# PengfeiRen96/DIR

Measured on AMD Instinct MI355X. Metric: images/sec at 256x256 bs=64, 3 stage outputs (DIR.forward eval), higher is better.
Workload: dtype f16

## Files before the change

dir_amd/_capi.py:

```python
import ctypes as C
import os

_HERE = os.path.dirname(os.path.abspath(__file__))
LIB_PATH = os.environ.get('DIR_LIB_PATH') or os.path.join(_HERE, 'lib', 'libdir_hip.so')
_lib = None


class DirHipError(RuntimeError):
    pass


class ManoTables(C.Structure):
    _fields_ = [('shapedirs_t', C.c_void_p), ('posedirs_t', C.c_void_p), ('v_template', C.c_void_p),
                ('j_template', C.c_void_p), ('j_shapedirs', C.c_void_p), ('weights', C.c_void_p), ('hands_mean', C.c_void_p),
                ('comps', C.c_void_p), ('side', C.c_int32), ('center_idx', C.c_int32), ('root_palm', C.c_int32)]


class ConvDesc(C.Structure):
    _fields_ = [(n, C.c_int32) for n in (
        'B', 'H', 'W', 'Cin', 'in_cstride', 'in_coff', 'Cout', 'out_cstride', 'out_coff', 'res_cstride', 'res_coff',
        'kh', 'kw', 'stride', 'pad', 'in_dtype', 'out_dtype', 'flags', 'Ho', 'Wo')] + [('in_scale', C.c_float), ('out_split_scale', C.c_float)]


class ConvBnBwd(C.Structure):
    _fields_ = [(n, C.c_void_p) for n in ('z', 'mean', 'rstd', 'w', 'b')] + [('relu', C.c_int32)] + [(n, C.c_void_p) for n in ('p1', 'p2')]


class ConvSrc2(C.Structure):
    _fields_ = [(n, C.c_int32) for n in ('H', 'W', 'Cin', 'in_cstride', 'in_coff', 'stride')]


class TrainWeight(C.Structure):
    _fields_ = [(n, C.c_void_p) for n in ('w', 'fwd', 'fwd_scale', 'dgrad', 'dgrad_scale')] + [(n, C.c_int32) for n in ('Cout', 'Cin', 'kh', 'kw')] + [
        ('fwd_inv_in', C.c_float), ('dgrad_inv_in', C.c_float)]


class BneckChainParams(C.Structure):
    _fields_ = [(n, C.c_void_p) for n in ('w2', 'scale2', 'shift2', 'w3', 'scale3', 'shift3', 'w1n', 'scale1n', 'shift1n', 'wd')] + [
        ('n_next', C.c_int32), ('out_decimate', C.c_int32), ('dtype', C.c_int32)]


class BneckTailParams(C.Structure):
    _fields_ = [(n, C.c_void_p) for n in ('wstream', 'scale3', 'shift3', 'scale1n', 'shift1n')] + [('planes', C.c_int32), ('n_next', C.c_int32), ('waves', C.c_int32), ('dtype', C.c_int32)]


class GemmDesc(C.Structure):
    _fields_ = [(n, C.c_int32) for n in ('M', 'N', 'K', 'lda', 'ldb', 'ldc', 'trans_a', 'trans_b', 'accumulate', 'batch')] + \
               [(n, C.c_int64) for n in ('stride_a', 'stride_b', 'stride_c')]


class GemmGroups(C.Structure):
    _fields_ = [(n, C.c_int32) for n in ('ny', 'nx', 'reduce', 'reserved')] + [(n, C.c_int64) for n in ('a_y', 'a_x', 'b_y', 'b_x', 'c_y', 'c_x')]


class TokenMlp(C.Structure):
    _fields_ = [(n, C.c_void_p) for n in ('w1t', 's1', 'b1', 'w2t', 'b2')]


class PgcnLayer(C.Structure):
    _fields_ = [(n, C.c_void_p) for n in ('W', 'e1', 'bias', 'bn_scale', 'bn_shift')] + [('relu', C.c_int32), ('w_dtype', C.c_int32)]


class SteBlock(C.Structure):
    _fields_ = [(n, C.c_void_p) for n in ('ln1_w', 'ln1_b', 'qkv_wt', 'qkv_b', 'proj_wt', 'proj_b', 'ln2_w', 'ln2_b',
                                          'fc1_wt', 'fc1_b', 'fc2_wt', 'fc2_b')]


class SteParams(C.Structure):
# ... 22 lines not shown


class LossPred(C.Structure):
    _fields_ = [('joint_uv', C.c_void_p * 2), ('mesh_uv', C.c_void_p * 2), ('proj', C.c_void_p * 2), ('joint_xyz', C.c_void_p * 2),
                ('mesh_xyz', C.c_void_p * 2), ('offset', C.c_void_p)]


class LossTarget(C.Structure):
    _fields_ = [('joint_2d', C.c_void_p * 2), ('mesh_2d', C.c_void_p * 2), ('joint_3d', C.c_void_p * 2),
                ('mesh_3d', C.c_void_p * 2), ('center', C.c_void_p * 2), ('faces', C.c_void_p * 2),
                ('c2', C.c_int32), ('n_faces', C.c_int32)]


class LossPredGrad(C.Structure):
    _fields_ = [('joint_uv', C.c_void_p * 2), ('mesh_uv', C.c_void_p * 2), ('joint_xyz', C.c_void_p * 2),
                ('mesh_xyz', C.c_void_p * 2), ('offset', C.c_void_p)]


class EvalOutputs(C.Structure):
    _fields_ = [(n, C.c_void_p) for n in ('joint_err', 'vert_err', 'joint2d_err', 'vert2d_err', 'joints_pd', 'joints_gt',
                                          'root_err')]


ABI_VERSION = 39
DT_F32, DT_BF16, DT_F16X3, DT_F16X1, DT_F16X3P, DT_F16X1P, DT_F16 = 0, 1, 3, 4, 5, 6, 7
CONV_RELU, CONV_PRE_RELU = 1, 2

_p, _i = C.c_void_p, C.c_int
_SIGNATURES = {
    'dir_abi_version': (C.c_int, []),
    'dir_last_error': (C.c_char_p, []),
    'dir_device_info': (C.c_int, [C.c_char_p, _i, C.POINTER(C.c_int)]),
    'dir_launch_log_reset': (None, []),
    'dir_launch_log_get': (C.c_int, [C.c_char_p, _i]),
    'dir_launch_log_note': (None, [C.c_char_p, C.c_longlong]),
    'dir_probe_launch': (C.c_longlong, [_i, _p, C.c_longlong, _i, _p]),
    'dir_conv2d_forward': (C.c_int, [C.POINTER(ConvDesc), _p, _p, _p, _p, _p, _p, _p, _p, _p]),
    'dir_conv2d_forward_stats': (C.c_int, [C.POINTER(ConvDesc), _p, _p, _p, _p, _p, _p, _p, _p, _p, C.POINTER(C.c_int), _p]),
    'dir_conv2d_forward_masked': (C.c_int, [C.POINTER(ConvDesc), _p, _p, _p, _p, _p, _p, _p, _p, _p, _p]),
    'dir_conv2d_forward_ex': (C.c_int, [C.POINTER(ConvDesc), _p, _p, _p, _p, _p, _p, _p, _p, _p, C.POINTER(ConvBnBwd), C.POINTER(C.c_int), _p]),
    'dir_add_upsampled': (C.c_int, [_p, _p, _i, _i, _i, _i, _i, _i, _i, _p]),
    'dir_fuse_sum': (C.c_int, [_p, _p, _p, _p, _i, _i, _i, _i, _i, _i, _i, _p]),
    'dir_pack_f16x3_weights': (C.c_int, [_p, _p, _p, _p, _i, _i, _p]),
    'dir_train_pack_conv_weights': (C.c_int, [_p, _p, _i, _i, _p]),
    'dir_gemm_f32_splitk_workspace_bytes': (C.c_longlong, [C.POINTER(GemmDesc)]),
    'dir_gemm_f32_splitk': (C.c_int, [C.POINTER(GemmDesc), _p, _p, _p, _p, _p, C.c_longlong, _p]),
    'dir_axpy_multi_f32': (C.c_int, [_p, _p, _p, _i, C.c_float, _p]),
    'dir_split_f16_forward': (C.c_int, [_p, _p, C.c_longlong, _i, _i, _i, _p, _p, _i, C.c_float, _i, _p]),
    'dir_stem_prep': (C.c_int, [_p, _p, _i, _i, _i, _i, _i, _i, _i, _p]),
    'dir_stem_prep_s2d': (C.c_int, [_p, _p, _i, _i, _i, _i, _i, _i, _p]),
    'dir_image_normalize_forward': (C.c_int, [_p, _p, C.POINTER(C.c_float), C.POINTER(C.c_float), _i, _i, _i, _p]),
    'dir_stem_prep_s2d_u8': (C.c_int, [_p, _p, C.POINTER(C.c_float), C.POINTER(C.c_float), _i, _i, _i, _i, _i, _i, _p]),
    'dir_adamw_step': (C.c_int, [_p, _p, _p, _p, C.c_longlong, C.c_double, C.c_double, C.c_double, C.c_double, C.c_double,
                                 C.c_longlong, _p]),
    'dir_stage_losses_backward': (C.c_int, [C.POINTER(LossPred), C.POINTER(LossTarget), C.c_float, _p, C.POINTER(C.c_void_p * 2),
                                            C.POINTER(C.c_void_p * 2), C.POINTER(LossPredGrad), _i, _p]),
    'dir_dense_losses_backward_workspace_bytes': (C.c_longlong, [_i, _i]),
    'dir_dense_losses_backward': (C.c_int, [_p, _p, _p, _p, C.POINTER(C.c_float), C.c_float, _p, _p, C.c_longlong, _p, _p, _i, _i, _i, _i, _p]),
    'dir_stage_losses_forward': (C.c_int, [C.POINTER(LossPred), C.POINTER(LossTarget), C.c_float, _p, _p, _i, _p]),
    'dir_dense_losses_workspace_bytes': (C.c_longlong, [_i, _i]),
    'dir_dense_losses_forward': (C.c_int, [_p, _p, _p, _p, C.POINTER(C.c_float), C.c_float, _p, C.c_longlong, _p, _i, _i, _i, _i, _p]),
    'dir_bottleneck_chain_forward': (C.c_int, [C.POINTER(BneckChainParams), _p, _p, _p, _p, _p, _i, _i, _i, _p]),
    'dir_bottleneck_tail_forward': (C.c_int, [C.POINTER(BneckTailParams), _p, _p, _p, _p, C.c_longlong, _p]),
    'dir_stem_pool_forward': (C.c_int, [_p, _i, C.POINTER(C.c_float), C.POINTER(C.c_float), _p, _p, _p, _p, _i, _i, _i, _p]),
    'dir_stem_pool_forward_dt': (C.c_int, [_p, _i, _i, C.POINTER(C.c_float), C.POINTER(C.c_float), _p, _p, _p, _p, _i, _i, _i, _p]),
    'dir_maxpool3x3s2': (C.c_int, [_p, _p, _i, _i, _i, _i, _i, _p]),
    'dir_upsample2x_bilinear': (C.c_int, [_p, _p, _i, _i, _i, _i, _i, _i, _i, _p]),
    'dir_init_head_forward': (C.c_int, [C.POINTER(InitHeadParams), _p, _p, _p, _i, _p, _p, _p, _i, _i, _i, _i, _i, _p]),
    'dir_bone_proj_forward': (C.c_int, [_p, _p, _p, _p, _p, _p, _i, _i, C.c_float, _i, _p]),
    'dir_conv2d_dual_forward': (C.c_int, [C.POINTER(ConvDesc), _p, C.POINTER(ConvSrc2), _p, _p, _p, _p, _p]),
    'dir_conv2d_dual_scaled_forward': (C.c_int, [C.POINTER(ConvDesc), _p, C.POINTER(ConvSrc2), _p, _p, _p, _p, _p, _p]),
    'dir_conv1x1_stream_forward': (C.c_int, [C.POINTER(ConvDesc), _p, C.POINTER(ConvSrc2), _p, _p, _p, _p, _p, _p, _p, _p]),
    'dir_conv2d_as_supported': (C.c_int, [C.POINTER(ConvDesc), _i, _i]),
    'dir_conv2d_as_forward': (C.c_int, [C.POINTER(ConvDesc), _p, _p, _p, _p, _p, _p, _i, _i, _p]),
    'dir_conv2d_sparse_forward': (C.c_int, [C.POINTER(ConvDesc), _p, _p, _p, _p, _p, _p, _p, _p]),
    'dir_grid_tokens_forward': (C.c_int, [_p, _i, _i, _i, _i, _i, _p, _p, _p, _p, _p, C.POINTER(TokenMlp),
                                          C.POINTER(TokenMlp), C.POINTER(TokenMlp), _p, _p, _i, _p]),
    'dir_pgcn_stack_forward': (C.c_int, [C.POINTER(PgcnLayer), _i, _p, _p, _p, C.c_longlong, _p, _i, _p]),
    'dir_pgcn_stack_forward_pair': (C.c_int, [C.POINTER(PgcnLayer), C.POINTER(PgcnLayer), _i, _p, _p, _p, _p, _i, _p]),
    'dir_pgcn_fused_sync_bytes': (C.c_longlong, []),
    'dir_pgcn_stack_forward_fused': (C.c_int, [C.POINTER(PgcnLayer), C.POINTER(PgcnLayer), _i, _p, _p, _p, _p, _p, _i, _i, _p]),
    'dir_ste_forward': (C.c_int, [C.POINTER(SteParams), _p, _p, _p, _i, _p]),
    'dir_regress_forward': (C.c_int, [C.POINTER(RegressParams), _p, _p, _p, _p, _p, _p, _p, _p, _i, _p]),
    'dir_bone_fusion_scratch_bytes': (C.c_size_t, [_i]),
    'dir_bone_fusion_prepare': (C.c_int, [C.POINTER(BoneFusionParams), _p, _p, _i, _p]),
    'dir_bone_fusion_forward': (C.c_int, [C.POINTER(BoneFusionParams), _p, _p, _p, _p, _i, _i, C.c_float, _i, _i, _i, _p]),
# ... 154 lines not shown
```

dir_amd/engine.py:

```python
import ctypes as C
import math
import json
import os
import threading

import torch

from . import _capi
from ._capi import CONV_PRE_RELU, CONV_RELU, DT_BF16, DT_F16, DT_F16X1, DT_F16X1P, DT_F16X3, DT_F16X3P, DT_F32, ConvDesc

F32 = torch.float32
IMAGENET_MEAN = (C.c_float * 3)(0.485, 0.456, 0.406)
IMAGENET_STD = (C.c_float * 3)(0.229, 0.224, 0.225)
_TLS = threading.local()


def _forced_variant():
    return getattr(_TLS, 'variant', None)


def _packing_arith():
    return getattr(_TLS, 'arith', None)


# ... 472 lines not shown
                and c1n.kh == 1 and c1n.stride == 1 and c1n.cin == c3.cout and c1n.scale is not None and c1n.pre_scale is None
                and (c3.cin, c1n.cout) in BneckTailOp.GEOMETRIES)

    def __call__(self, y2, x, out=None, y1n=None):
        B, H, W, P = y2.shape
        M = B * H * W
        if getattr(_TLS, 'capture_fused', None) is not None:
            _TLS.capture_fused.append((self, (y2, x), {}))
        if out is None:
            out = torch.empty(B, H, W, self.c3.cout, device=y2.device, dtype=y2.dtype)
        if y1n is None:
            y1n = torch.empty(B, H, W, self.c1n.cout, device=y2.device, dtype=y2.dtype)
        if _capi.PROFILE is not None:
            c4, n2 = self.c3.cout, self.c1n.cout
            _capi.annotate(family='conv', flops=2.0 * M * (P * c4 + c4 * n2), op=self, dtype='bf16',
                           shape='M=%d tail 1x1(%d->%d)+res+1x1(->%d)' % (M, P, c4, n2),
                           bytes=(M * (P + 2 * c4 + n2) + c4 * P + n2 * c4) * 2)
        waves = self.force_waves or (4 if M // 64 <= self.THIN_MAX_TILES else 8)
        _capi.check(_capi.lib().dir_bottleneck_tail_forward(C.byref(self.params[waves]), _capi.ptr(y2), _capi.ptr(x), _capi.ptr(out), _capi.ptr(y1n),
                                                            M, _capi.stream_ptr()), 'dir_bottleneck_tail_forward')
        return out, y1n


def stem_conv_op(w, scale, shift, dtype):
    wp = torch.zeros(64, 64, 4, 1, device=w.device, dtype=F32)
    for r in range(4):
        for dy in range(2):
            ky = 2 * r + dy - 1
            if not 0 <= ky <= 6:
                continue
            for j in range(4):
                for dx in range(2):
                    kx = 2 * j + dx - 1
                    if 0 <= kx <= 6:
                        c0 = j * 16 + (dy * 2 + dx) * 4
                        wp[:, c0:c0 + 3, r, 0] = w[:, :, ky, kx]
    op = ConvOp(wp, dtype, stride=1, pad=0, scale=scale, shift=shift, relu=True)
    op.ho = op.wo = 128
    op.in_cs_override = 16
    op.alg_k = 147
    return op


class BackboneOp(object):
    fold_downsample = os.environ.get('DIR_FOLD_DOWNSAMPLE', '1') != '0'
    fused_stem = os.environ.get('DIR_FUSED_STEM', '1') != '0'
# ... 32 lines not shown
                if 'dual' not in blk and blk['ds'] is None:
                    blk['c2'].link_split(blk['c3'])
                blocks.append(blk)
            self.layers.append(blocks)
        if self.bneck_chain:
            l1 = self.layers[0]
            for i, blk in enumerate(l1):
                nxt = l1[i + 1]['c1'] if i + 1 < len(l1) else self.layers[1][0]['c1']
                if 'dual' in blk:
                    if BneckChainOp.applies(blk['c2'], None, nxt, dt, dual=blk['dual']):
                        blk['chain'] = BneckChainOp(blk['c2'], None, nxt, dual=blk['dual'])
                elif blk['ds'] is None and BneckChainOp.applies(blk['c2'], blk['c3'], nxt, dt):
                    blk['chain'] = BneckChainOp(blk['c2'], blk['c3'], nxt)

        if self.bneck_tail:
            for li in (1, 2):
                blocks = self.layers[li]
                for i, blk in enumerate(blocks):
                    if 'dual' in blk or blk['ds'] is not None or 'chain' in blk:
                        continue
                    nxt = blocks[i + 1]['c1'] if i + 1 < len(blocks) else self.layers[li + 1][0]['c1']
                    if BneckTailOp.applies(blk['c3'], nxt, dt):
                        blk['tail'] = BneckTailOp(blk['c3'], nxt)

    def __call__(self, img):
        L, dt, dev = _capi.lib(), self.dtype, self.device
        B = img.shape[0]
        if self.fused_stem and dt in HALF:
            x = torch.empty(B, 64, 64, 64, device=dev, dtype=dt)
            u8 = img.dtype == torch.uint8
            _ann('stem', 2.0 * B * 128 * 128 * 64 * 147, img.numel() * img.element_size() + x.numel() * 2 + self.stem_w.numel() * 2,
                 'B=%d 7x7/2 conv + bn + relu + maxpool' % B)
            nb = self.subbatch
            last2 = self.layers[1][-1]
            if nb and nb < B and B % nb == 0 and 'tail' in last2 and not getattr(_TLS, 'capture_fused', None) and not getattr(_TLS, 'no_out_split', False):
                c2 = torch.empty(B, 32, 32, 512, device=dev, dtype=dt)
                y1n = torch.empty(B, 32, 32, last2['tail'].c1n.cout, device=dev, dtype=dt)
                _TLS.parent_batch = B
                try:
                    for b0 in range(0, B, nb):
                        isub = img[b0:b0 + nb]
                        xs = x[b0:b0 + nb]
                        _ann('stem', 2.0 * nb * 128 * 128 * 64 * 147, isub.numel() * isub.element_size() + xs.numel() * 2 + self.stem_w.numel() * 2,
                             'B=%d 7x7/2 conv + bn + relu + maxpool' % nb)
                        _capi.check(L.dir_stem_pool_forward_dt(_capi.ptr(isub), 2 if u8 else 0, _dt(dt), IMAGENET_MEAN, IMAGENET_STD, _capi.ptr(self.stem_w),
                                                            _capi.ptr(self.stem_scale), _capi.ptr(self.stem_shift), _capi.ptr(xs), nb, 256, 256,
# ... 17 lines not shown
                        'dir_stem_prep_s2d')
        s1 = self.stem(xp)
        x = torch.empty(B, 64, 64, 64, device=dev, dtype=dt)
        _ann('stem', 0, (s1.numel() + x.numel()) * x.element_size(), 'B=%d maxpool 3x3/2' % B)
        _capi.check(L.dir_maxpool3x3s2(_capi.ptr(s1), _capi.ptr(x), B, 128, 128, 64, _dt(dt), _capi.stream_ptr()),
                    'dir_maxpool3x3s2')
        return self._layers(x)

    decimate_c1 = os.environ.get('DIR_DECIMATE_C1', '1') != '0'
    subbatch = int(os.environ.get('DIR_SUBBATCH', '0'))

    def _layers(self, x, start=0, upto=4, y1=None, out_last=None):
        feats = []
        x_dec = False
        for li in range(start, upto):
            blocks = self.layers[li]
            for bi, blk in enumerate(blocks):
                if 'chain' in blk:
                    dec = (self.decimate_c1 and li == 0 and bi == len(blocks) - 1 and blk['chain'].c1n is not None and 'dual' in self.layers[1][0]
                           and self.layers[1][0]['dual'].stride2 == 2 and 'chain' not in self.layers[1][0] and not getattr(_TLS, 'no_out_split', False))
                    x, y1 = blk['chain'](y1 if y1 is not None else blk['c1'](x), x, decimate=dec)
                    x_dec = dec
                    continue
                if 'tail' in blk and (x.shape[0] * x.shape[1] * x.shape[2]) % 64 == 0:
                    if out_last is not None and li == upto - 1 and bi == len(blocks) - 1:
                        x, y1 = blk['tail'](blk['c2'](y1 if y1 is not None else blk['c1'](x)), x, out=out_last[0], y1n=out_last[1])
                        continue
                    x, y1 = blk['tail'](blk['c2'](y1 if y1 is not None else blk['c1'](x)), x)
                elif 'dual' in blk:
                    x, y1 = blk['dual'](blk['c2'](y1 if y1 is not None else blk['c1'](x)), x, x_decimated=x_dec), None
                    x_dec = False
                else:
                    idn = blk['ds'](x) if blk['ds'] is not None else x
                    x, y1 = blk['c3'](blk['c2'](y1 if y1 is not None else blk['c1'](x)), residual=idn), None
            feats.append(None if x_dec else x)
        return feats


def backbone_standalone(module, x, compute_dtype=torch.float32):
    _capi.require_cuda(x)
    if module.training:
        raise NotImplementedError('dir_amd implements the inference path (eval-mode BatchNorm); call .eval()')
    sd = {'b.' + k: v.detach() for k, v in module.state_dict().items()}
    op = BackboneOp(sd, 'b', compute_dtype, x.device)
    op.decimate_c1 = False
    with torch.cuda.device(x.device):
# ... 771 lines not shown
```

dir_amd/functional.py:

```python
import torch

from . import _capi
from ._capi import CONV_PRE_RELU, CONV_RELU, DT_BF16, DT_F16, DT_F16X1, DT_F16X1P, DT_F16X3, DT_F16X3P, DT_F32, ConvDesc


def _dt(t):
    if t.dtype == torch.float32:
        return DT_F32
    if t.dtype == torch.bfloat16:
        return DT_BF16
    if t.dtype == torch.float16:
        return DT_F16
    raise _capi.DirHipError('unsupported dtype %s' % t.dtype)


def pack_conv_weight(w_oihw, dtype=torch.float32):
    return w_oihw.detach().permute(0, 2, 3, 1).contiguous().to(dtype)


def pack_f16x3_weights(w_rows, scale=None):
    w = w_rows.detach().float()
    Cout, K = w.shape
    assert K % 32 == 0
    amax = w.abs().amax(1).cpu()
# ... 178 lines not shown
    import ctypes as C
    _capi.check(_capi.lib().dir_bottleneck_chain_forward(C.byref(p), _capi.ptr(y1), _capi.ptr(residual) if residual is not None else None,
                                                         _capi.ptr(dual[0]) if dual is not None else None, _capi.ptr(out), _capi.ptr(y1n) if y1n is not None else None, B, H, W,
                                                         _capi.stream_ptr()), 'dir_bottleneck_chain_forward')
    return out, y1n


def bottleneck_tail(y2, w3, s3, h3, residual, w1n, s1n, h1n, waves=8):
    import ctypes as C
    from .engine import pack_tail_stream
    _capi.require_cuda(y2, residual)
    B, H, W, P = y2.shape
    C4, N2 = w3.shape[0], w1n.shape[0]
    stream = pack_tail_stream(w3, w1n, waves, dtype=y2.dtype)
    keep = [_capi.f32c(t) for t in (s3, h3, s1n, h1n)]
    out = torch.empty(B, H, W, C4, device=y2.device, dtype=y2.dtype)
    y1n = torch.empty(B, H, W, N2, device=y2.device, dtype=y2.dtype)
    p = _capi.BneckTailParams(_capi.ptr(stream), _capi.ptr(keep[0]), _capi.ptr(keep[1]), _capi.ptr(keep[2]), _capi.ptr(keep[3]), P, N2, waves, _dt(y2))
    _capi.check(_capi.lib().dir_bottleneck_tail_forward(C.byref(p), _capi.ptr(y2.contiguous()), _capi.ptr(residual.contiguous()), _capi.ptr(out),
                                                        _capi.ptr(y1n), B * H * W, _capi.stream_ptr()), 'dir_bottleneck_tail_forward')
    return out, y1n


def conv1x1_stream(x, w_nk, scale=None, shift=None, relu=False, pre_scale=None, pre_shift=None, pre_relu=False, x2=None, stride2=1,
                   out=None, out_coff=0, in_coff=0, cin=None, variant=0):
    from .engine import pack_stream_weights
    _capi.require_cuda(x, x2, out)
    B, H, W, cbuf = x.shape
    Cout, K = w_nk.shape
    cin2 = x2.shape[3] if x2 is not None else 0
    cin = cin if cin is not None else K - cin2
    assert cin + cin2 == K
    ws = pack_stream_weights(w_nk, dtype=x.dtype)
    if out is None:
        out = torch.empty(B, H, W, Cout, device=x.device, dtype=x.dtype)
    d = ConvDesc(B, H, W, cin, cbuf, in_coff, Cout, out.shape[3], out_coff, 0, 0, 1, 1, 1, 0, _dt(x), _dt(out),
                 (CONV_RELU if relu else 0) | (CONV_PRE_RELU if pre_relu else 0) | ((variant & 0xff) << 8))
    d2 = _capi.ConvSrc2(x2.shape[1], x2.shape[2], cin2, x2.shape[3], 0, stride2) if x2 is not None else None
    keep = [None if t is None else _capi.f32c(t) for t in (scale, shift, pre_scale, pre_shift)]
    _capi.check(_capi.lib().dir_conv1x1_stream_forward(d, _capi.ptr(x), d2, _capi.ptr(x2), _capi.ptr(ws), _capi.ptr(keep[0]), _capi.ptr(keep[1]),
                                                       _capi.ptr(keep[2]), _capi.ptr(keep[3]), _capi.ptr(out), _capi.stream_ptr()),
                'dir_conv1x1_stream_forward')
    return out


def mano_backward(tables_lr, para_lr, g_verts=None, g_joints=None, g_joint_uv=None, g_mesh_uv=None):
# ... 36 lines not shown
```

include/dir_hip.h:

```cpp
#ifndef DIR_HIP_H
#define DIR_HIP_H

#include <stddef.h>
#include <stdint.h>

#ifdef __cplusplus
extern "C" {
#endif

#define DIR_OK 0
#define DIR_E_INVALID (-1)
#define DIR_E_LAUNCH (-2)
#define DIR_E_NODEVICE (-3)

#define DIR_ABI_VERSION 39

int dir_abi_version(void);
const char* dir_last_error(void);
int dir_device_info(char* arch_host, int arch_len, int* num_cu_host);
void dir_launch_log_reset(void);
int dir_launch_log_get(char* buf_host, int len);
void dir_launch_log_note(const char* name, long long times);
long long dir_probe_launch(int mode, void* buf, long long bytes, int iters, void* stream);

typedef struct dir_mano_tables {
    const float* shapedirs_t;
    const float* posedirs_t;
    const float* v_template;
    const float* j_template;
    const float* j_shapedirs;
    const float* weights;
    const float* hands_mean;
    const float* comps;
    int32_t side;
    int32_t center_idx;
    int32_t root_palm;
} dir_mano_tables;

// ... 323 lines not shown
    const void* w2; const float* scale2; const float* shift2;
    const void* w3; const float* scale3; const float* shift3;
    const void* w1n; const float* scale1n; const float* shift1n;
    const void* wd;
    int32_t n_next;
    int32_t out_decimate;
    int32_t dtype;
} dir_bneck_chain_params;
int dir_bottleneck_chain_forward(const dir_bneck_chain_params* p, const void* y1, const void* residual, const void* x2, void* out,
                                 void* y1_next, int B, int H, int W, void* stream);

typedef struct dir_bneck_tail_params {
    const void* wstream;
    const float* scale3; const float* shift3;
    const float* scale1n; const float* shift1n;
    int32_t planes;
    int32_t n_next;
    int32_t waves;
    int32_t dtype;
} dir_bneck_tail_params;
int dir_bottleneck_tail_forward(const dir_bneck_tail_params* p, const void* y2, const void* residual, void* out, void* y1_next,
                                long long M, void* stream);

typedef struct dir_loss_pred {
    const float* joint_uv[2];
    const float* mesh_uv[2];
    const float* proj[2];
    const float* joint_xyz[2];
    const float* mesh_xyz[2];
    const float* offset;
} dir_loss_pred;
typedef struct dir_loss_target {
    const float* joint_2d[2];
    const float* mesh_2d[2];
    const float* joint_3d[2];
    const float* mesh_3d[2];
    const float* center[2];
    const int32_t* faces[2];
    int32_t c2, n_faces;
} dir_loss_target;
int dir_stage_losses_forward(const dir_loss_pred* pred_host, const dir_loss_target* gt_host, float coord_weight, double* scratch,
                             float* out13, int B, void* stream);
long long dir_dense_losses_workspace_bytes(int B, int S);
int dir_dense_losses_forward(const float* seg_logits, const float* dense_pred, const float* gt_seg, const float* gt_dense,
                             const float* class_weight_host, float dense_weight, void* workspace, long long workspace_bytes,
                             float* out3, int B, int S, int H, int W, void* stream);
// ... 54 lines not shown
```

Before: 26720.

## Fuse bottleneck 3x3 conv, 1x1 expand, residual and next 1x1 into one kernel

Adds a persistent HIP kernel that runs a whole ResNet bottleneck body per 64-pixel tile. It loads the y1 patch into LDS via DMA, does the 3x3 conv with MFMA, keeps y2 in LDS, then applies the 1x1 expansion with BN, residual add and ReLU, and optionally the next block's 1x1 conv. The aim is to remove the HBM round trip of the y2 intermediate and some launches for layers 1 and 2. In exchange it uses heavy LDS and register pressure with one block per CU, which may limit latency hiding compared with the separate tuned kernels.

```diff
diff --git a/dir_amd/_capi.py b/dir_amd/_capi.py
--- a/dir_amd/_capi.py
+++ b/dir_amd/_capi.py
@@ -44,6 +44,11 @@
     _fields_ = [(n, C.c_void_p) for n in ('wstream', 'scale3', 'shift3', 'scale1n', 'shift1n')] + [('planes', C.c_int32), ('n_next', C.c_int32), ('waves', C.c_int32), ('dtype', C.c_int32)]
 
 
+class BneckBlockParams(C.Structure):
+    _fields_ = [(n, C.c_void_p) for n in ('w2stream', 'wstream', 'scale2', 'shift2', 'scale3', 'shift3', 'scale1n', 'shift1n')] + [
+        ('planes', C.c_int32), ('n_next', C.c_int32), ('stride', C.c_int32), ('dtype', C.c_int32)]
+
+
 class GemmDesc(C.Structure):
     _fields_ = [(n, C.c_int32) for n in ('M', 'N', 'K', 'lda', 'ldb', 'ldc', 'trans_a', 'trans_b', 'accumulate', 'batch')] + \
                [(n, C.c_int64) for n in ('stride_a', 'stride_b', 'stride_c')]
@@ -112,7 +117,7 @@
                                           'root_err')]
 
 
-ABI_VERSION = 39
+ABI_VERSION = 40
 DT_F32, DT_BF16, DT_F16X3, DT_F16X1, DT_F16X3P, DT_F16X1P, DT_F16 = 0, 1, 3, 4, 5, 6, 7
 CONV_RELU, CONV_PRE_RELU = 1, 2
 
@@ -152,6 +157,7 @@
     'dir_dense_losses_forward': (C.c_int, [_p, _p, _p, _p, C.POINTER(C.c_float), C.c_float, _p, C.c_longlong, _p, _i, _i, _i, _i, _p]),
     'dir_bottleneck_chain_forward': (C.c_int, [C.POINTER(BneckChainParams), _p, _p, _p, _p, _p, _i, _i, _i, _p]),
     'dir_bottleneck_tail_forward': (C.c_int, [C.POINTER(BneckTailParams), _p, _p, _p, _p, C.c_longlong, _p]),
+    'dir_bottleneck_block_forward': (C.c_int, [C.POINTER(BneckBlockParams), _p, _p, _p, _p, C.c_int, C.c_int, C.c_int, _p]),
     'dir_stem_pool_forward': (C.c_int, [_p, _i, C.POINTER(C.c_float), C.POINTER(C.c_float), _p, _p, _p, _p, _i, _i, _i, _p]),
     'dir_stem_pool_forward_dt': (C.c_int, [_p, _i, _i, C.POINTER(C.c_float), C.POINTER(C.c_float), _p, _p, _p, _p, _i, _i, _i, _p]),
     'dir_maxpool3x3s2': (C.c_int, [_p, _p, _i, _i, _i, _i, _i, _p]),
diff --git a/dir_amd/csrc/bneck_block.hip b/dir_amd/csrc/bneck_block.hip
--- /dev/null
+++ b/dir_amd/csrc/bneck_block.hip
@@ -0,0 +1,399 @@
+#include "conv_common.h"
+
+namespace dir {
+namespace {
+
+using convk::bf16_t;
+using convk::f16s_t;
+using convk::f32x16;
+using convk::Half;
+typedef __attribute__((ext_vector_type(4))) float f32x4;
+
+constexpr unsigned OOB = 0x80000000u;
+constexpr int TM = 64;
+constexpr int HC = 512;
+constexpr int NTHR = 512;
+constexpr int TPITCH = HC * 2 + 16;
+
+struct BlockArgs {
+    const bf16_t* y1; const bf16_t* res; bf16_t* out; bf16_t* y1n;
+    const uint4* w2s;
+    const uint4* wstream;
+    const float* sc2; const float* sh2; const float* sc3; const float* sh3; const float* sc1n; const float* sh1n;
+    int ntiles, H, tiles_per_img; unsigned y1_bytes;
+};
+
+template <typename H> __device__ __forceinline__ void unpack4(uint2 v, float (&f)[4]) {
+    convk::unpack2<H>(v.x, f[0], f[1]);
+    convk::unpack2<H>(v.y, f[2], f[3]);
+}
+
+template <int P, int N2, typename H = bf16_t>
+__global__ __launch_bounds__(NTHR, 1) void block_tail_chain_kernel(BlockArgs a) {
+    convk::half_kernel_init<H>();
+    constexpr int C4 = 4 * P, NH = C4 / HC;
+    constexpr int YROW = P * 2;
+    constexpr int GRP = P == 256 ? 4 : 8;
+    constexpr int KBS = P / 16;
+    constexpr int NBF = 2 * KBS;
+    constexpr bool HAS_NEXT = N2 > 0;
+    constexpr bool C16 = N2 == 128;
+    constexpr int NCF = !HAS_NEXT ? 0 : C16 ? HC / 32 : HC / 16;
+    constexpr int NF = NBF + NCF, NG = NF / GRP;
+    static_assert(NF % GRP == 0 && NG % 2 == 0 && C4 % HC == 0 && (N2 == 0 || N2 == 128 || N2 == 256) && (P == 128 || P == 256),
+                  "block_tail_chain_kernel: unsupported geometry");
+    constexpr int W = P == 128 ? 32 : 16, LOGW = P == 128 ? 5 : 4, TR = TM / W, PW = W + 2, NPOS = (TR + 2) * PW;
+    constexpr int Q = P / 8;
+    constexpr int PITCH = 2 * P + 16;
+    constexpr int NINSTR = (NPOS * (Q + 1) + 63) / 64;
+    constexpr int PATCH_BYTES = NINSTR * 1024;
+    constexpr int NSTEP = 9 * P / 64;
+    constexpr int PBN = P == 256 ? 2 : 1;
+    constexpr int NSTG = 3;
+    constexpr bool OVERLAY = P == 256;
+    constexpr int T_BYTES = TM * TPITCH;
+    constexpr int PT_BYTES = OVERLAY ? (T_BYTES > PATCH_BYTES ? T_BYTES : PATCH_BYTES) : T_BYTES + PATCH_BYTES;
+    __shared__ __attribute__((aligned(16))) char s_pt[PT_BYTES];
+    __shared__ __attribute__((aligned(16))) char s_y2[TM * YROW];
+    __shared__ __attribute__((aligned(16))) float s_ss[2 * P + 2 * C4 + 2 * (HAS_NEXT ? N2 : 4)];
+    char* const s_t = s_pt;
+    char* const s_patch = OVERLAY ? s_pt : s_pt + T_BYTES;
+    constexpr int SS3 = 2 * P, SS1 = 2 * P + 2 * C4;
+    const int tid = threadIdx.x, lane = tid & 63, wave = __builtin_amdgcn_readfirstlane(tid >> 6);
+    const int l32 = lane & 31, h = lane >> 5, l16 = lane & 15, g16 = lane >> 4;
+
+    for (int i = tid; i < P; i += NTHR) { s_ss[i] = a.sc2[i]; s_ss[P + i] = a.sh2[i]; }
+    for (int i = tid; i < C4; i += NTHR) { s_ss[SS3 + i] = a.sc3[i]; s_ss[SS3 + C4 + i] = a.sh3[i]; }
+    if constexpr (HAS_NEXT) {
+        for (int i = tid; i < N2; i += NTHR) { s_ss[SS1 + i] = a.sc1n[i]; s_ss[SS1 + N2 + i] = a.sh1n[i]; }
+    }
+
+    const int tstep = gridDim.x;
+    int t = blockIdx.x;
+    if (t >= a.ntiles) return;
+
+    const convk::i32x4 yd = {(int)(unsigned)(unsigned long long)a.y1, (int)(unsigned)((unsigned long long)a.y1 >> 32), (int)a.y1_bytes, 0x00020000};
+    const unsigned patch_lds = (unsigned)(unsigned long long)(__attribute__((address_space(3))) char*)&s_pt[0] + (OVERLAY ? 0u : (unsigned)T_BYTES);
+    auto patch_dma = [&](int tile) {
+        const int img = tile / a.tiles_per_img, trow = (tile - img * a.tiles_per_img) * TR;
+#pragma unroll
+        for (int j = 0; j < (NINSTR + 7) / 8; ++j) {
+            const int i = wave + 8 * j;
+            if (i < NINSTR) {
+                const int slot = i * 64 + lane, pos = slot / (Q + 1), ch = slot - pos * (Q + 1);
+                const int pr = pos / PW, pc = pos - pr * PW;
+                const int iy = trow + pr - 1, ix = pc - 1;
+                const bool ok = pos < NPOS && ch < Q && (unsigned)iy < (unsigned)a.H && (unsigned)ix < (unsigned)W;
+                const unsigned voff = ok ? (unsigned)((((img * a.H + iy) * W + ix) * P) * 2 + (ch << 4)) : OOB;
+                convk::lds_dma16_m0(yd, (unsigned)__builtin_amdgcn_readfirstlane((int)(patch_lds + (unsigned)i * 1024u)), voff, 0);
+            }
+        }
+    };
+    uint4 xr[2][2][2];
+    auto res_fetch = [&](int tile, int half) {
+#pragma unroll
+        for (int pb = 0; pb < 2; ++pb) {
+            const bf16_t* rp = a.res + ((long long)tile * TM + 32 * pb + l32) * C4 + half * HC + 64 * wave + 8 * h;
+#pragma unroll
+            for (int cb = 0; cb < 2; ++cb)
+#pragma unroll
+                for (int j = 0; j < 2; ++j) xr[cb][pb][j] = *reinterpret_cast<const uint4*>(rp + 32 * cb + 16 * j);
+        }
+    };
+    uint4 ring[2][GRP];
+    auto ring_load = [&](auto Slot, int hf, int grp) {
+        constexpr int slot = decltype(Slot)::value;
+        const uint4* p = a.wstream + ((long long)(hf * 8 + wave) * NF + grp * GRP) * 64 + lane;
+#pragma unroll
+        for (int i = 0; i < GRP; ++i) ring[slot][i] = p[i * 64];
+    };
+
+    const int cbA = P == 256 ? wave : (wave >> 1);
+    int pixA[PBN], posb[PBN];
+    {
+        const bool g1 = ((l32 >= 4) & (l32 < 12)) | ((l32 >= 16) & (l32 < 20)) | (l32 >= 28);
+        const int rk = g1 ? (l32 < 12 ? l32 - 4 : l32 < 20 ? l32 - 8 : l32 - 16) : (l32 < 4 ? l32 : l32 < 16 ? l32 - 8 : l32 - 12);
+#pragma unroll
+        for (int j = 0; j < PBN; ++j) {
+            const int pb = PBN == 2 ? j : (wave & 1);
+            const int p = 16 * (2 * pb + (g1 ? 1 : 0)) + rk;
+            pixA[j] = p;
+            posb[j] = ((p >> LOGW) * PW + (p & (W - 1))) * PITCH + 64 * h;
+        }
+    }
+    const uint4* w2p = a.w2s + (long long)cbA * (NSTEP * 4 * 64) + lane;
+
+    patch_dma(t);
+    ring_load(std::integral_constant<int, 0>{}, 0, 0);
+    res_fetch(t, 0);
+
+    f32x16 accb[2];
+    f32x16 accc32[(C16 || !HAS_NEXT) ? 1 : 2];
+    f32x4 accc16[C16 ? 4 : 1];
+    constexpr int NOP = C16 ? 4 : 2;
+    uint4 bop[2][NOP];
+    auto act_read = [&](auto F, auto Set) {
+        constexpr int f = decltype(F)::value, set = decltype(Set)::value;
+        if constexpr (f < NBF) {
+            constexpr int ks = f % KBS;
+#pragma unroll
+            for (int pb = 0; pb < 2; ++pb)
+                bop[set][pb] = *reinterpret_cast<const uint4*>(s_y2 + (32 * pb + l32) * YROW + (((HAS_NEXT ? 2 * ks + h : 8 * (ks / 4) + (ks % 4) + 4 * h) ^ (l32 & 15)) << 4));
+        } else {
+            constexpr int fc = f - NBF;
+            if constexpr (C16) {
+#pragma unroll
+                for (int u = 0; u < 4; ++u) bop[set][u] = *reinterpret_cast<const uint4*>(s_t + (16 * u + l16) * TPITCH + 64 * fc + 16 * g16);
+            } else {
+#pragma unroll
+                for (int pb = 0; pb < 2; ++pb) bop[set][pb] = *reinterpret_cast<const uint4*>(s_t + (32 * pb + l32) * TPITCH + 32 * fc + 16 * h);
+            }
+        }
+    };
+
+    for (; t < a.ntiles; t += tstep) {
+        const bool more = t + tstep < a.ntiles;
+        {
+            uint4 wr[NSTG][4];
+            auto wload = [&](auto Stage, int step) {
+                constexpr int stage = decltype(Stage)::value;
+                const uint4* wp = w2p + (long long)min(step, NSTEP - 1) * 256;
+#pragma unroll
+                for (int ks = 0; ks < 4; ++ks) wr[stage][ks] = wp[ks * 64];
+            };
+            [&]<int... S>(std::integer_sequence<int, S...>) { (wload(std::integral_constant<int, S>{}, S), ...); }(std::make_integer_sequence<int, NSTG - 1>{});
+            convk::wait_vmcnt<0>();
+            __syncthreads();
+            f32x16 acc[PBN];
+#pragma unroll
+            for (int j = 0; j < PBN; ++j)
+#pragma unroll
+                for (int r = 0; r < 16; ++r) acc[j][r] = 0.f;
+            uint4 bv[4][PBN];
+            auto bread = [&](auto KK, const char* base) {
+                constexpr int kk = decltype(KK)::value, k = kk % 36, tap = k / 4, ks = k % 4, ky = tap / 3, kx = tap - 3 * ky;
+                constexpr int soff = (ky * PW + kx) * PITCH + 16 * ks + (kk >= 36 ? 128 : 0);
+#pragma unroll
+                for (int j = 0; j < PBN; ++j) bv[ks][j] = *reinterpret_cast<const uint4*>(base + posb[j] + soff);
+            };
+            bread(std::integral_constant<int, 0>{}, s_patch);
+            bread(std::integral_constant<int, 1>{}, s_patch);
+#pragma unroll 1
+            for (int slab = 0; slab < P / 64; ++slab) {
+                const char* base = s_patch + slab * 128;
+                [&]<int... T>(std::integer_sequence<int, T...>) {
+                    (([&] {
+                         constexpr int tap = T, stage = tap % NSTG;
+                         wload(std::integral_constant<int, (tap + NSTG - 1) % NSTG>{}, slab * 9 + tap + NSTG - 1);
+                         [&]<int... KS>(std::integer_sequence<int, KS...>) {
+                             (([&] {
+                                  bread(std::integral_constant<int, 4 * tap + KS + 2>{}, base);
+#pragma unroll
+                                  for (int j = 0; j < PBN; ++j) acc[j] = Half<H>::mfma32(wr[stage][KS], bv[KS][j], acc[j]);
+                              }()),
+                              ...);
+                         }(std::make_integer_sequence<int, 4>{});
+                     }()),
+                     ...);
+                }(std::make_integer_sequence<int, 9>{});
+            }
+#pragma unroll
+            for (int q = 0; q < 4; ++q) {
+                const int c0 = 32 * cbA + 8 * q + 4 * h;
+                const float4 sc = *reinterpret_cast<const float4*>(s_ss + c0);
+                const float4 sh = *reinterpret_cast<const float4*>(s_ss + P + c0);
+#pragma unroll
+                for (int j = 0; j < PBN; ++j) {
+                    uint2 o;
+                    o.x = Half<H>::pack2_relu(fmaf(acc[j][4 * q], sc.x, sh.x), fmaf(acc[j][4 * q + 1], sc.y, sh.y));
+                    o.y = Half<H>::pack2_relu(fmaf(acc[j][4 * q + 2], sc.z, sh.z), fmaf(acc[j][4 * q + 3], sc.w, sh.w));
+                    *reinterpret_cast<uint2*>(s_y2 + pixA[j] * YROW + ((((c0 >> 3) ^ (pixA[j] & 15))) << 4) + 8 * h) = o;
+                }
+            }
+        }
+        __syncthreads();
+        if constexpr (!OVERLAY) {
+            if (more) patch_dma(t + tstep);
+        }
+#pragma nounroll
+        for (int hf = 0; hf < NH; ++hf) {
+            const bool last_half = hf == NH - 1;
+            if constexpr (HAS_NEXT) {
+                if (hf == 0) {
+                    if constexpr (C16) {
+#pragma unroll
+                        for (int u = 0; u < 4; ++u) accc16[u] = f32x4{0.f, 0.f, 0.f, 0.f};
+                    } else {
+#pragma unroll
+                        for (int pb = 0; pb < 2; ++pb)
+#pragma unroll
+                            for (int r = 0; r < 16; ++r) accc32[pb][r] = 0.f;
+                    }
+                }
+            }
+            act_read(std::integral_constant<int, 0>{}, std::integral_constant<int, 0>{});
+            [&]<int... G>(std::integer_sequence<int, G...>) {
+                (([&] {
+                     constexpr int grp = G, slot = G & 1;
+                     if constexpr (grp + 1 < NG) ring_load(std::integral_constant<int, slot ^ 1>{}, hf, grp + 1);
+                     else ring_load(std::integral_constant<int, slot ^ 1>{}, last_half ? 0 : hf + 1, 0);
+                     [&]<int... I>(std::integer_sequence<int, I...>) {
+                         (([&] {
+                              constexpr int f = grp * GRP + I, set = f & 1;
+                              if constexpr (f + 1 < NF && f + 1 != NBF) act_read(std::integral_constant<int, f + 1>{}, std::integral_constant<int, set ^ 1>{});
+                              if constexpr (f < NBF) {
+                                  constexpr int cb = f / KBS, ks = f - cb * KBS;
+                                  if constexpr (ks == 0) {
+#pragma unroll
+                                      for (int pb = 0; pb < 2; ++pb)
+#pragma unroll
+                                          for (int r = 0; r < 16; ++r) accb[pb][r] = 0.f;
+                                  }
+#pragma unroll
+                                  for (int pb = 0; pb < 2; ++pb)
+                                      accb[pb] = Half<H>::mfma32(ring[slot][I], bop[set][pb], accb[pb]);
+                                  if constexpr (ks == KBS - 1) {
+#pragma unroll
+                                      for (int q = 0; q < 4; ++q) {
+                                          const int cl = 64 * wave + 32 * cb + 8 * q + 4 * h;
+                                          const float4 sc = *reinterpret_cast<const float4*>(s_ss + SS3 + hf * HC + cl);
+                                          const float4 sh = *reinterpret_cast<const float4*>(s_ss + SS3 + C4 + hf * HC + cl);
+#pragma unroll
+                                          for (int pb = 0; pb < 2; ++pb) {
+                                              float v[4] = {fmaf(accb[pb][4 * q], sc.x, sh.x), fmaf(accb[pb][4 * q + 1], sc.y, sh.y),
+                                                            fmaf(accb[pb][4 * q + 2], sc.z, sh.z), fmaf(accb[pb][4 * q + 3], sc.w, sh.w)};
+                                              float rv[4];
+                                              {
+                                                  const uint4 c = xr[cb][pb][q >> 1];
+                                                  const auto sx = __builtin_amdgcn_permlane32_swap(c.x, c.z, false, false);
+                                                  const auto sy = __builtin_amdgcn_permlane32_swap(c.y, c.w, false, false);
+                                                  unpack4<H>(make_uint2(sx[q & 1], sy[q & 1]), rv);
+                                              }
+#pragma unroll
+                                              for (int e = 0; e < 4; ++e) v[e] += rv[e];
+                                              uint2 o;
+                                              o.x = Half<H>::pack2_relu(v[0], v[1]);
+                                              o.y = Half<H>::pack2_relu(v[2], v[3]);
+                                              *reinterpret_cast<uint2*>(s_t + (32 * pb + l32) * TPITCH + cl * 2) = o;
+                                          }
+                                          __builtin_amdgcn_sched_barrier(0);
+                                      }
+                                  }
+                                  if constexpr (f == NBF - 1) {
+                                      __syncthreads();
+                                      if constexpr (HAS_NEXT) act_read(std::integral_constant<int, NBF>{}, std::integral_constant<int, set ^ 1>{});
+                                      if (!last_half) res_fetch(t, hf + 1);
+                                      else res_fetch(more ? t + tstep : t, 0);
+#pragma unroll
+                                      for (int i = 0; i < TM * (HC / 8) / NTHR; ++i) {
+                                          const int c = tid + NTHR * i;
+                                          *reinterpret_cast<uint4*>(a.out + ((long long)t * TM + (c >> 6)) * C4 + hf * HC + (c & 63) * 8) =
+                                              *reinterpret_cast<const uint4*>(s_t + (c >> 6) * TPITCH + (c & 63) * 16);
+                                          if (i & 1) __builtin_amdgcn_sched_barrier(0);
+                                      }
+                                  }
+                              } else {
+                                  if constexpr (C16) {
+#pragma unroll
+                                      for (int u = 0; u < 4; ++u)
+                                          accc16[u] = Half<H>::mfma16(ring[slot][I], bop[set][u], accc16[u]);
+                                  } else {
+#pragma unroll
+                                      for (int pb = 0; pb < 2; ++pb)
+                                          accc32[pb] = Half<H>::mfma32(ring[slot][I], bop[set][pb], accc32[pb]);
+                                  }
+                              }
+                              __builtin_amdgcn_sched_barrier(0);
+                          }()),
+                          ...);
+                     }(std::make_integer_sequence<int, GRP>{});
+                 }()),
+                 ...);
+            }(std::make_integer_sequence<int, NG>{});
+            if constexpr (HAS_NEXT) {
+                if (last_half) {
+                    if constexpr (C16) {
+                        const int c0 = 16 * wave + 4 * g16;
+                        const float4 sc = *reinterpret_cast<const float4*>(s_ss + SS1 + c0);
+                        const float4 sh = *reinterpret_cast<const float4*>(s_ss + SS1 + N2 + c0);
+#pragma unroll
+                        for (int u = 0; u < 4; ++u) {
+                            uint2 o;
+                            o.x = Half<H>::pack2_relu(fmaf(accc16[u][0], sc.x, sh.x), fmaf(accc16[u][1], sc.y, sh.y));
+                            o.y = Half<H>::pack2_relu(fmaf(accc16[u][2], sc.z, sh.z), fmaf(accc16[u][3], sc.w, sh.w));
+                            *reinterpret_cast<uint2*>(a.y1n + ((long long)t * TM + 16 * u + l16) * N2 + c0) = o;
+                        }
+                    } else {
+#pragma unroll
+                        for (int pb = 0; pb < 2; ++pb) {
+                            uint2 o[4];
+#pragma unroll
+                            for (int q = 0; q < 4; ++q) {
+                                const int c0 = 32 * wave + 8 * q + 4 * h;
+                                const float4 sc = *reinterpret_cast<const float4*>(s_ss + SS1 + c0);
+                                const float4 sh = *reinterpret_cast<const float4*>(s_ss + SS1 + N2 + c0);
+                                o[q].x = Half<H>::pack2_relu(fmaf(accc32[pb][4 * q], sc.x, sh.x), fmaf(accc32[pb][4 * q + 1], sc.y, sh.y));
+                                o[q].y = Half<H>::pack2_relu(fmaf(accc32[pb][4 * q + 2], sc.z, sh.z), fmaf(accc32[pb][4 * q + 3], sc.w, sh.w));
+                            }
+#pragma unroll
+                            for (int j = 0; j < 2; ++j) {
+                                const auto dx = __builtin_amdgcn_permlane32_swap(o[2 * j].x, o[2 * j + 1].x, false, false);
+                                const auto dy = __builtin_amdgcn_permlane32_swap(o[2 * j].y, o[2 * j + 1].y, false, false);
+                                *reinterpret_cast<uint4*>(a.y1n + ((long long)t * TM + 32 * pb + l32) * N2 + 32 * wave + 16 * j + 8 * h) = make_uint4(dx[0], dy[0], dx[1], dy[1]);
+                            }
+                        }
+                    }
+                }
+            }
+            __syncthreads();
+        }
+        if constexpr (OVERLAY) {
+            if (more) patch_dma(t + tstep);
+        }
+    }
+}
+
+}
+}
+
+extern "C" int dir_bottleneck_block_forward(const dir_bneck_block_params* p, const void* y1, const void* residual, void* out, void* y1_next,
+                                            int B, int H, int W, void* stream) {
+    using namespace dir;
+    DIR_REQUIRE(p && y1 && residual && out, "dir_bottleneck_block_forward: null pointer");
+    DIR_REQUIRE(p->w2stream && p->wstream && p->scale2 && p->shift2 && p->scale3 && p->shift3, "dir_bottleneck_block_forward: missing parameters");
+    DIR_REQUIRE(p->stride == 1, "dir_bottleneck_block_forward: stride must be 1 (identity bottlenecks only)");
+    DIR_REQUIRE(p->planes == 128 || p->planes == 256, "dir_bottleneck_block_forward: planes must be 128 or 256");
+    DIR_REQUIRE(B > 0 && H > 0 && W == (p->planes == 128 ? 32 : 16) && ((long long)H * W) % TM == 0,
+                "dir_bottleneck_block_forward: W must be 32 (planes 128) or 16 (planes 256) and H * W a multiple of 64");
+    const bool next = y1_next != nullptr;
+    DIR_REQUIRE(next == (p->n_next != 0), "dir_bottleneck_block_forward: y1_next and n_next must be given together");
+    DIR_REQUIRE(!next || (p->scale1n && p->shift1n), "dir_bottleneck_block_forward: y1_next needs the next conv1's scale / shift");
+    DIR_REQUIRE(p->n_next == 0 || p->n_next == 256 || (p->n_next == 128 && p->planes == 128),
+                "dir_bottleneck_block_forward: n_next must be 0, 128 (planes 128) or 256");
+    DIR_REQUIRE(p->dtype == 0 || p->dtype == DIR_DT_BF16 || p->dtype == DIR_DT_F16, "dir_bottleneck_block_forward: dtype must be bf16 (or 0) or f16");
+    const long long M = (long long)B * H * W;
+    DIR_REQUIRE(M * p->planes * 2 < (1ll << 31), "dir_bottleneck_block_forward: y1 must be < 2 GiB (32-bit buffer offsets)");
+    const bool f16 = p->dtype == DIR_DT_F16;
+    BlockArgs a;
+    a.y1 = (const convk::bf16_t*)y1; a.res = (const convk::bf16_t*)residual; a.out = (convk::bf16_t*)out; a.y1n = (convk::bf16_t*)y1_next;
+    a.w2s = (const uint4*)p->w2stream; a.wstream = (const uint4*)p->wstream;
+    a.sc2 = p->scale2; a.sh2 = p->shift2; a.sc3 = p->scale3; a.sh3 = p->shift3; a.sc1n = p->scale1n; a.sh1n = p->shift1n;
+    a.ntiles = (int)(M / TM); a.H = H; a.tiles_per_img = H * W / TM;
+    a.y1_bytes = (unsigned)(M * p->planes * 2);
+    static int num_cu = 0;
+    if (!num_cu) {
+        int dev = 0; hipDeviceProp_t pr;
+        num_cu = (hipGetDevice(&dev) == hipSuccess && hipGetDeviceProperties(&pr, dev) == hipSuccess) ? pr.multiProcessorCount : 256;
+    }
+    const int grid = a.ntiles < num_cu ? a.ntiles : num_cu;
+    hipStream_t s = (hipStream_t)stream;
+#define DIR_BLOCK(P_, N2_) do { if (f16) DIR_LAUNCH((block_tail_chain_kernel<P_, N2_, f16s_t>), dim3(grid), dim3(NTHR), 0, s, a); \
+                                 else DIR_LAUNCH((block_tail_chain_kernel<P_, N2_, bf16_t>), dim3(grid), dim3(NTHR), 0, s, a); } while (0)
+    if (p->planes == 128 && p->n_next == 0) DIR_BLOCK(128, 0);
+    else if (p->planes == 128 && p->n_next == 128) DIR_BLOCK(128, 128);
+    else if (p->planes == 128 && p->n_next == 256) DIR_BLOCK(128, 256);
+    else if (p->planes == 256 && p->n_next == 0) DIR_BLOCK(256, 0);
+    else DIR_BLOCK(256, 256);
+#undef DIR_BLOCK
+    return check_launch("dir_bottleneck_block_forward");
+}
diff --git a/dir_amd/engine.py b/dir_amd/engine.py
--- a/dir_amd/engine.py
+++ b/dir_amd/engine.py
@@ -518,6 +518,84 @@
         return out, y1n
 
 
+def pack_block_conv2_stream(w2_ohwi):
+    N, kh, kw, Cin = w2_ohwi.shape
+    assert kh == 3 and kw == 3 and N % 32 == 0 and Cin % 64 == 0
+    dev = w2_ohwi.device
+    w = w2_ohwi.reshape(N, 9 * Cin)
+    lane = torch.arange(64, device=dev)
+    l32, h = lane & 31, lane >> 5
+    e = torch.arange(8, device=dev)
+    cb, st, ks = torch.meshgrid(torch.arange(N // 32, device=dev), torch.arange(9 * Cin // 64, device=dev), torch.arange(4, device=dev), indexing='ij')
+    row = (cb * 32)[..., None] + l32
+    slab, tap = st // 9, st % 9
+    k0 = (tap * Cin + 64 * slab + 8 * ks)[..., None] + 32 * h
+    return w[row[..., None], k0[..., None] + e].contiguous()
+
+
+def pack_block_conv3_stream(w3, dtype=torch.bfloat16):
+    out_dev = w3.device
+    w3 = w3.detach().float().reshape(w3.shape[0], -1).cpu()
+    C4, P = w3.shape
+    assert C4 == 4 * P and C4 % 512 == 0
+    lane = torch.arange(64)
+    l32, h = lane & 31, lane >> 5
+    e = torch.arange(8)
+    out = []
+    for hf in range(C4 // 512):
+        for w in range(8):
+            for cb in range(2):
+                for ks in range(P // 16):
+                    out.append(w3[(hf * 512 + 64 * w + 32 * cb + l32)[:, None], (64 * (ks // 4) + 8 * (ks % 4) + 32 * h)[:, None] + e])
+    return torch.stack(out).to(dtype).contiguous().to(out_dev)
+
+
+class BneckBlockOp(object):
+    WIDTH = {128: 32, 256: 16}
+    _env = os.environ.get('DIR_BNECK_BLOCK', '1')
+    PLANES = () if _env == '0' else (128, 256) if _env == '1' else tuple(int(v) for v in _env.split(','))
+
+    def __init__(self, c2, c3, c1n=None, tail=None):
+        self.c2, self.c3, self.c1n = c2, c3, c1n
+        self.cout, self.cin, self.kh, self.kw, self.stride = c3.cout, c2.cin, 3, 3, 1
+        self.variant = {}
+        self.w2s = pack_block_conv2_stream(c2.w)
+        self.stream = tail.stream[8] if tail is not None else pack_block_conv3_stream(c3.w.reshape(c3.cout, c3.cin), dtype=c3.dtype)
+        n = (lambda t: None) if c1n is None else _capi.ptr
+        self.params = _capi.BneckBlockParams(_capi.ptr(self.w2s), _capi.ptr(self.stream), _capi.ptr(c2.scale), _capi.ptr(c2.shift),
+                                             _capi.ptr(c3.scale), _capi.ptr(c3.shift), n(c1n.scale if c1n is not None else None),
+                                             n(c1n.shift if c1n is not None else None), c2.cin, c1n.cout if c1n is not None else 0, c2.stride, _dt(c2.dtype))
+
+    @staticmethod
+    def applies(c2, c3, c1n, dtype):
+        ok = (dtype in HALF and c2.kh == 3 and c2.kw == 3 and c2.stride == 1 and c2.pad == 1 and c2.cin == c2.cout and c2.cin in BneckBlockOp.PLANES
+              and c2.scale is not None and c2.pre_scale is None and c3.kh == 1 and c3.stride == 1 and c3.cin == c2.cout and c3.cout == 4 * c3.cin
+              and c3.scale is not None)
+        return ok and (c1n is None or (c1n.kh == 1 and c1n.stride == 1 and c1n.cin == c3.cout and c1n.scale is not None and c1n.pre_scale is None
+                                       and (c3.cin, c1n.cout) in BneckTailOp.GEOMETRIES))
+
+    def fits(self, y1):
+        return y1.shape[2] == self.WIDTH[self.c2.cin] and (y1.shape[1] * y1.shape[2]) % 64 == 0 and y1.is_contiguous()
+
+    def __call__(self, y1, x, out=None, y1n=None):
+        B, H, W, P = y1.shape
+        M = B * H * W
+        if getattr(_TLS, 'capture_fused', None) is not None:
+            _TLS.capture_fused.append((self, (y1, x), {}))
+        if out is None:
+            out = torch.empty(B, H, W, self.c3.cout, device=y1.device, dtype=y1.dtype)
+        if y1n is None and self.c1n is not None:
+            y1n = torch.empty(B, H, W, self.c1n.cout, device=y1.device, dtype=y1.dtype)
+        if _capi.PROFILE is not None:
+            c4, n2 = self.c3.cout, self.c1n.cout if self.c1n is not None else 0
+            _capi.annotate(family='conv', flops=2.0 * M * (9 * P * P + P * c4 + c4 * n2), op=self, dtype='bf16',
+                           shape='M=%d block 3x3(%d)+1x1(->%d)+res%s' % (M, P, c4, '+1x1(->%d)' % n2 if n2 else ''),
+                           bytes=(M * (P + 2 * c4 + n2) + 9 * P * P + c4 * P + n2 * c4) * 2)
+        _capi.check(_capi.lib().dir_bottleneck_block_forward(C.byref(self.params), _capi.ptr(y1), _capi.ptr(x), _capi.ptr(out), _capi.ptr(y1n),
+                                                             B, H, W, _capi.stream_ptr()), 'dir_bottleneck_block_forward')
+        return out, y1n
+
+
 def stem_conv_op(w, scale, shift, dtype):
     wp = torch.zeros(64, 64, 4, 1, device=w.device, dtype=F32)
     for r in range(4):
@@ -596,6 +674,13 @@
                     nxt = blocks[i + 1]['c1'] if i + 1 < len(blocks) else self.layers[li + 1][0]['c1']
                     if BneckTailOp.applies(blk['c3'], nxt, dt):
                         blk['tail'] = BneckTailOp(blk['c3'], nxt)
+        for li in (1, 2):
+            for blk in self.layers[li]:
+                if 'dual' in blk or blk['ds'] is not None or 'chain' in blk:
+                    continue
+                nxt = blk['tail'].c1n if 'tail' in blk else None
+                if ('tail' in blk or li == 2) and BneckBlockOp.applies(blk['c2'], blk['c3'], nxt, dt):
+                    blk['block'] = BneckBlockOp(blk['c2'], blk['c3'], nxt, tail=blk.get('tail'))
 
     def __call__(self, img):
         L, dt, dev = _capi.lib(), self.dtype, self.device
@@ -659,6 +744,13 @@
                     x, y1 = blk['chain'](y1 if y1 is not None else blk['c1'](x), x, decimate=dec)
                     x_dec = dec
                     continue
+                if 'block' in blk:
+                    ya = y1 if y1 is not None else blk['c1'](x)
+                    if blk['block'].fits(ya):
+                        last = out_last is not None and li == upto - 1 and bi == len(blocks) - 1
+                        x, y1 = blk['block'](ya, x, out=out_last[0] if last else None, y1n=out_last[1] if last else None)
+                        continue
+                    y1 = ya
                 if 'tail' in blk and (x.shape[0] * x.shape[1] * x.shape[2]) % 64 == 0:
                     if out_last is not None and li == upto - 1 and bi == len(blocks) - 1:
                         x, y1 = blk['tail'](blk['c2'](y1 if y1 is not None else blk['c1'](x)), x, out=out_last[0], y1n=out_last[1])
diff --git a/dir_amd/functional.py b/dir_amd/functional.py
--- a/dir_amd/functional.py
+++ b/dir_amd/functional.py
@@ -224,6 +224,28 @@
     return out, y1n
 
 
+def bottleneck_block(y1, w2, s2, h2, w3, s3, h3, residual, nxt=None, stride=1, out=None, y1n=None):
+    import ctypes as C
+    from .engine import pack_block_conv2_stream, pack_block_conv3_stream, pack_tail_stream
+    _capi.require_cuda(y1, residual)
+    B, H, W, P = y1.shape
+    C4 = w3.shape[0]
+    N2 = nxt[0].shape[0] if nxt is not None else 0
+    w2s = pack_block_conv2_stream(w2.to(y1.dtype).contiguous())
+    stream = pack_tail_stream(w3, nxt[0], 8, dtype=y1.dtype) if nxt is not None else pack_block_conv3_stream(w3, dtype=y1.dtype)
+    keep = [_capi.f32c(t) for t in (s2, h2, s3, h3)] + ([_capi.f32c(nxt[1]), _capi.f32c(nxt[2])] if nxt is not None else [None, None])
+    if out is None:
+        out = torch.empty(B, H, W, C4, device=y1.device, dtype=y1.dtype)
+    if y1n is None and nxt is not None:
+        y1n = torch.empty(B, H, W, N2, device=y1.device, dtype=y1.dtype)
+    assert out.is_contiguous() and (y1n is None or y1n.is_contiguous())
+    p = _capi.BneckBlockParams(_capi.ptr(w2s), _capi.ptr(stream), _capi.ptr(keep[0]), _capi.ptr(keep[1]), _capi.ptr(keep[2]), _capi.ptr(keep[3]),
+                               _capi.ptr(keep[4]) if nxt is not None else None, _capi.ptr(keep[5]) if nxt is not None else None, P, N2, stride, _dt(y1))
+    _capi.check(_capi.lib().dir_bottleneck_block_forward(C.byref(p), _capi.ptr(y1.contiguous()), _capi.ptr(residual.contiguous()), _capi.ptr(out),
+                                                         _capi.ptr(y1n) if y1n is not None else None, B, H, W, _capi.stream_ptr()), 'dir_bottleneck_block_forward')
+    return out, y1n
+
+
 def conv1x1_stream(x, w_nk, scale=None, shift=None, relu=False, pre_scale=None, pre_shift=None, pre_relu=False, x2=None, stride2=1,
                    out=None, out_coff=0, in_coff=0, cin=None, variant=0):
     from .engine import pack_stream_weights
diff --git a/include/dir_hip.h b/include/dir_hip.h
--- a/include/dir_hip.h
+++ b/include/dir_hip.h
@@ -13,7 +13,7 @@
 #define DIR_E_LAUNCH (-2)
 #define DIR_E_NODEVICE (-3)
 
-#define DIR_ABI_VERSION 39
+#define DIR_ABI_VERSION 40
 
 int dir_abi_version(void);
 const char* dir_last_error(void);
@@ -383,6 +383,19 @@
 int dir_bottleneck_tail_forward(const dir_bneck_tail_params* p, const void* y2, const void* residual, void* out, void* y1_next,
                                 long long M, void* stream);
 
+typedef struct dir_bneck_block_params {
+    const void* w2stream; const void* wstream;
+    const float* scale2; const float* shift2;
+    const float* scale3; const float* shift3;
+    const float* scale1n; const float* shift1n;
+    int32_t planes;
+    int32_t n_next;
+    int32_t stride;
+    int32_t dtype;
+} dir_bneck_block_params;
+int dir_bottleneck_block_forward(const dir_bneck_block_params* p, const void* y1, const void* residual, void* out, void* y1_next,
+                                 int B, int H, int W, void* stream);
+
 typedef struct dir_loss_pred {
     const float* joint_uv[2];
     const float* mesh_uv[2];
```

Measured after the change: 25700, median of 2. -3.8%, worse.
